# autonomousvision/ppo.cpp

Measured on AMD Instinct MI355X. Metric: env steps/sec (SPS), HalfCheetah-v5 num_envs=4096 at 1/2/4/8 MI355X, higher is better.
Workload: dtype f32

## Files before the change

### include/ppo_hip.h

```cpp
#ifndef PPO_HIP_H
#define PPO_HIP_H

#include <stddef.h>
#include <stdint.h>

#include "ppo_layout.h"

#ifdef __cplusplus
extern "C" {
#endif

typedef struct ppo_ctx ppo_t;

typedef struct ppo_hip_config {
  int net_kind;
  int obs_dim, act_dim;
  int hidden;
  int num_envs;
  int num_steps;
  int num_minibatches;
  int update_epochs;
  float gamma, gae_lambda;
  float clip_coef, ent_coef, vf_coef, max_grad_norm, adam_eps;
  int norm_adv, clip_vloss;
// ... 35 lines not shown
                             void* stream);
int ppo_get_value(ppo_t* ctx, int n, const float* x_dev, float* value_dev, void* stream);

int ppo_rollout_act(ppo_t* ctx, int step, int env_begin, int env_end, const float* next_obs_dev,
                    const float* next_done_dev, float* action_out_dev, void* stream);
int ppo_rollout_values(ppo_t* ctx, void* stream);
int ppo_rollout_reward(ppo_t* ctx, int step, int env_begin, int env_end, const float* reward_dev, void* stream);
int ppo_compute_gae(ppo_t* ctx, const float* next_obs_dev, const float* next_done_dev, int num_steps_collected,
                    void* stream);
int ppo_gae_from_values(ppo_t* ctx, const float* next_value_dev, const float* next_done_dev, int num_steps_collected,
                        void* stream);
int ppo_update(ppo_t* ctx, float lr, const int32_t* perms_dev, ppo_update_stats* stats);
int ppo_update_ex(ppo_t* ctx, float lr, int num_steps_collected, const int32_t* perms_dev, ppo_update_stats* stats);
int ppo_sync(ppo_t* ctx);
int ppo_debug_last_grad(ppo_t* ctx, float* host, long n);
int ppo_snapshot_state(ppo_t* ctx);
int ppo_read_snapshot(ppo_t* ctx, float* params_host, float* m_host, float* v_host, long n, long* step);
long ppo_iteration(const ppo_t* ctx);
int ppo_set_iteration(ppo_t* ctx, long iteration);
float* ppo_buffer(ppo_t* ctx, int which);

#define PPO_COMM_ID_BYTES 128
int ppo_comm_unique_id(char id_out[PPO_COMM_ID_BYTES]);
int ppo_comm_init(ppo_t* ctx, const char id[PPO_COMM_ID_BYTES], int rank, int world);
typedef int (*ppo_host_allreduce_fn)(float* host_buf, long n, int average, void* user);
int ppo_comm_init_host(ppo_t* ctx, int rank, int world, ppo_host_allreduce_fn fn, void* user);
int ppo_comm_destroy(ppo_t* ctx);
int ppo_comm_broadcast_params(ppo_t* ctx, int root);
int ppo_comm_allreduce(ppo_t* ctx, float* buf_dev, long n, int average);
enum { PPO_COMM_NONE = 0, PPO_COMM_RCCL = 1, PPO_COMM_HOST = 2 };
int ppo_comm_info(const ppo_t* ctx, int* kind, int* rank, int* world);
int ppo_get_device(const ppo_t* ctx, int* device, char* pci_bus_id, int len);
int ppo_kernel_info(const ppo_t* ctx, char* buf, int len);

int ppo_set_device(int device);
int ppo_device_count(int* n);
int ppo_dev_malloc(void** p, size_t bytes);
int ppo_dev_free(void* p);
int ppo_memcpy_h2d(void* dst_dev, const void* src_host, size_t bytes);
int ppo_memcpy_d2h(void* dst_host, const void* src_dev, size_t bytes);
int ppo_memset_dev(void* dst_dev, int value, size_t bytes);
int ppo_device_sync(void);

int ppo_profile_enable(ppo_t* ctx, int on);
int ppo_profile_read(ppo_t* ctx, double* ms, long* count, int cap);
const char* ppo_profile_name(int id);
int ppo_profile_reset(ppo_t* ctx);

#ifdef __cplusplus
}
#endif
#endif
```

### ppo.cpp_amd/csrc/ppo_capi.hip

```cpp
#include <hip/hip_runtime.h>
#include <rccl/rccl.h>

#include <dlfcn.h>
#include <link.h>
#include <unistd.h>

#include <algorithm>
#include <atomic>
#include <cmath>
#include <cstdio>
#include <cstdlib>
#include <cstring>
#include <mutex>
#include <string>
#include <vector>

#include "../../include/ppo_hip.h"
#include "../../include/ppo_synth_env.h"
#include "../../include/ppo_env_wrappers.h"
#include "ppo_kernels.hpp"

static thread_local std::string g_err;
static int fail(const std::string& msg, int code = -1) {
  g_err = msg;
// ... 112 lines not shown
  int upd32_mix = 0;
  bool use_upd2 = false;
  int rollout_kernel = 0;
  int upd2_split = 0;
  float* Z1 = nullptr;
  UpdGeoOut upd = {};
  int upd_nblk = 0;
  size_t lds_bytes = 0;
  int wlds_off = 0;
  float* dwslab[4] = {};
  int nchunks = 1, rows_per_chunk = 64, dw_slices = 1;
  float* normout = nullptr;
  float* gnpart = nullptr;
  float* cs_sq = nullptr;
  unsigned* cs_cnt = nullptr;
  int gn_fold = 0;
  float* mbstats = nullptr;
  float* snap = nullptr;
  hipEvent_t snap_ev = nullptr;
  hipStream_t snap_stream = nullptr;
  long snap_step = 0;
  long adam_step = 0;
  long iteration = 0;
  ncclComm_t comm = nullptr;
  ppo_host_allreduce_fn host_ar = nullptr;
  void* host_user = nullptr;
  std::vector<float> host_stage;
  int world = 1, rank = 0;
  int act_kernel = 0;
  int upd_trunk_mask = 3, upd_sched = 1;
  int dw_fused = 1;
  int dw_dma = 1;
  int dw_bx = 0;
  int rollout_mode = PPO_ROLLOUT_AUTO;
  int gradstep = 0;
  unsigned* gs_bar = nullptr;
  unsigned gs_count = 0;
  int update_graph = 0;
  bool update_graph_auto = false;
  hipGraphExec_t upd_exec = nullptr;
  const int32_t* upd_exec_perms = nullptr;
  long upd_calls = 0;
  float* sched = nullptr;
  float* sched_host[2] = {};
  hipEvent_t sched_ev[2] = {};
  int sched_flip = 0;
  float* beta_store = nullptr;
  unsigned prof_mask = 0;
  std::mutex prof_mu;
  std::vector<ProfEvent> pending;
  std::vector<hipEvent_t> free_events;
  double prof_ms[PK_COUNT] = {};
  long prof_cnt[PK_COUNT] = {};
};

static hipEvent_t prof_event(ppo_t* c) {
  if (!c->free_events.empty()) {
    hipEvent_t e = c->free_events.back();
    c->free_events.pop_back();
    return e;
  }
  hipEvent_t e;
  (void)hipEventCreate(&e);
  return e;
}
struct ProfScope {
// ... 28 lines not shown
    c->free_events.push_back(p.a);
    c->free_events.push_back(p.b);
  }
  c->pending.clear();
}

static hipStream_t S(ppo_t* c, void* s) { return s ? (hipStream_t)s : c->stream; }
static void comm_detach(ppo_t* c);

template <typename T>
static int dmalloc(T** p, size_t n) {
  if (n == 0) n = 1;
  hipError_t e = hipMalloc((void**)p, n * sizeof(T));
  if (e != hipSuccess) return fail(std::string("hipMalloc: ") + hipGetErrorString(e), -2);
  (void)hipMemset(*p, 0, n * sizeof(T));
  return 0;
}

struct CreateOptions {
  int upd_kernel = 0;
  int act_kernel = 0;
  int dw_fused = 1;
  int rollout = PPO_ROLLOUT_AUTO;
  int gradstep = 0;
  int gradnorm = -1;
  int dw_rows = 0;
  int dw_slices = 0;
  int dw_dma = 1;
  int dw_bx = -1;
  int gae_scan = -1;
  int values_mfma = -1;
  int upd_split = 0;
  int h1_handoff = -1;
  int update_graph = -1;
  int rollout_kernel = 0;
  int upd2_split = -1;
  int upd_mfma = 0;
};
static constexpr int kUpd2SplitAuto = 0;
static constexpr int kDwBxAuto = 6;
static constexpr int kUpdBxAuto = 1;
static constexpr int kUpd2BxAuto = 1;
static constexpr int kGaeScanMinT = 512;
static int kUpdSplitAuto(int M) { (void)M; return 1; }
static constexpr bool kH1RecomputeAuto = false;
static constexpr int kUpdGraphAutoRows = 4096;
static constexpr int kGradnormFoldAuto = 0;
static int parse_create_options(const char* opts, CreateOptions* o) {
  if (!opts) return 0;
  std::string s(opts);
  size_t pos = 0;
  while (pos < s.size()) {
    size_t end = s.find(',', pos);
    if (end == std::string::npos) end = s.size();
    const std::string kv = s.substr(pos, end - pos);
    pos = end + 1;
    if (kv.empty()) continue;
    const size_t eq = kv.find('=');
    if (eq == std::string::npos) return fail("ppo_create_ex: option without '=': " + kv);
    const std::string k = kv.substr(0, eq), v = kv.substr(eq + 1);
    if (k == "upd_kernel" && (v == "auto" || v == "fwdbwd")) o->upd_kernel = v == "fwdbwd";
    else if (k == "act_kernel" && (v == "auto" || v == "2" || v == "4")) o->act_kernel = v == "auto" ? 0 : v[0] - '0';
    else if (k == "dw_fused" && (v == "0" || v == "1")) o->dw_fused = v[0] - '0';
    else if (k == "rollout" && (v == "auto" || v == "per_step"))
      o->rollout = v == "auto" ? PPO_ROLLOUT_AUTO : PPO_ROLLOUT_PER_STEP;
    else if (k == "gradstep" && (v == "fused" || v == "split")) o->gradstep = v == "fused";
    else if (k == "gradnorm" && (v == "auto" || v == "slices" || v == "fold")) o->gradnorm = v == "auto" ? -1 : v == "fold";
    else if (k == "dw_rows" && !v.empty() && v.size() <= 5 && v.find_first_not_of("0123456789") == std::string::npos &&
             atoi(v.c_str()) % 16 == 0 && atoi(v.c_str()) >= 16 && atoi(v.c_str()) <= 65536)
      o->dw_rows = atoi(v.c_str());
    else if (k == "dw_slices" && (v == "1" || v == "2")) o->dw_slices = v[0] - '0';
    else if (k == "dw_dma" && (v == "0" || v == "1")) o->dw_dma = v[0] - '0';
    else if (k == "gae" && (v == "auto" || v == "serial" || v == "scan")) o->gae_scan = v == "auto" ? -1 : v == "scan";
    else if (k == "h1_handoff" && (v == "auto" || v == "store" || v == "recompute"))
      o->h1_handoff = v == "auto" ? -1 : v == "recompute";
    else if (k == "upd_split" && (v == "auto" || v == "1" || v == "2" || v == "4" || v == "8"))
      o->upd_split = v == "auto" ? 0 : v[0] - '0';
    else if (k == "values_mfma" && (v == "auto" || v == "f32" || v == "bx6"))
      o->values_mfma = v == "auto" ? -1 : v == "f32" ? 0 : 6;
    else if (k == "dw_mfma" && (v == "auto" || v == "f32" || v == "bf16x9" || v == "bf16x8" || v == "bf16x6"))
      o->dw_bx = v == "auto" ? -1 : v == "f32" ? 0 : v == "bf16x9" ? 9 : v == "bf16x8" ? 8 : 6;
    else if (k == "update_graph" && (v == "auto" || v == "0" || v == "1")) o->update_graph = v == "auto" ? -1 : v[0] - '0';
    else if (k == "rollout_kernel" && (v == "auto" || v == "mfma" || v == "valu"))
      o->rollout_kernel = v == "auto" ? 0 : v == "mfma" ? 1 : 2;
    else if (k == "upd2_split" && (v == "auto" || v == "0" || v == "2" || v == "3")) o->upd2_split = v == "auto" ? -1 : v[0] - '0';
    else if (k == "upd_mfma" && (v == "auto" || v == "16" || v == "32" || v == "mix" || v == "bx6"))
      o->upd_mfma = v == "auto" ? 0 : v == "mix" ? 1 : v == "bx6" ? 6 : atoi(v.c_str());
    else return fail("ppo_create_ex: unknown option or value: " + kv);
  }
  return 0;
}

extern "C" int ppo_create(const ppo_hip_config* cfg, int device, ppo_t** out) {
  return ppo_create_ex(cfg, device, nullptr, out);
}

extern "C" int ppo_create_ex(const ppo_hip_config* cfg, int device, const char* options, ppo_t** out) {
  if (!cfg || !out) return fail("ppo_create: null argument");
  CreateOptions opt;
  if (parse_create_options(options, &opt)) return -1;
  if (int rc = ppo_runtime_check()) return rc;
  ppo_layout L;
  if (ppo_layout_init(&L, cfg->net_kind, cfg->obs_dim, cfg->act_dim, cfg->hidden) != 0)
    return fail("ppo_create: bad net kind / dims");
  if (cfg->hidden != 64 && cfg->hidden != 256) return fail("ppo_create: hidden must be 64 or 256");
  if (cfg->act_dim > 20) return fail("ppo_create: act_dim > 20 not supported");
  if (cfg->num_envs <= 0 || cfg->num_steps <= 0 || cfg->num_minibatches <= 0 || cfg->update_epochs <= 0)
    return fail("ppo_create: sizes must be positive");
// ... 164 lines not shown
      if (opt.upd_split > 1) {
        ppo_destroy(c);
        return fail("ppo_create: upd_split > 1 needs the fused k_upd + k_dwf path (hidden 256, obs_dim <= 32)");
      }
      S = 1;
    }
    while (S > 1 && c->M < S * 32 * 64) S /= 2;
    c->msplit = S;
    c->Mq = S == 1 ? c->M : (((c->M + S - 1) / S + 31) & ~31);
    while (c->msplit > 1 && (long)(c->msplit - 1) * c->Mq >= c->M) --c->msplit;
  }
  for (int k = 0; k < 2; ++k)
    rc |= dmalloc(&c->slab[k], (size_t)c->msplit * std::max(c->nblk, c->upd_nblk) * c->sg[k].size);
  c->wlds_off = 4 * std::max(c->sg[0].size, c->sg[1].size);
  c->wlds_off = (c->wlds_off + 63) & ~63;
  c->lds_bytes = ((size_t)c->wlds_off + 2 * (size_t)H * 16) * sizeof(float);
  c->dw_slices = dw_slices(c->Mq, H, OP, true);
  if (opt.dw_slices && H == 256 && OP <= 32) c->dw_slices = opt.dw_slices;
  c->rows_per_chunk = std::max(64, (((c->Mq + 128 / c->dw_slices - 1) / (128 / c->dw_slices)) + 15) & ~15);
  if (c->use_upd2) c->rows_per_chunk = std::max(32, (((c->M + 255) / 256) + 31) & ~31);
  if (opt.dw_rows && (!c->use_upd2 || opt.dw_rows % 32 == 0)) c->rows_per_chunk = opt.dw_rows;
  c->nchunks = (c->Mq + c->rows_per_chunk - 1) / c->rows_per_chunk;
  {
    const bool rc_ok = c->use_upd && !c->use_upd2 && !c->use_upd32 && cfg->net_kind == PPO_NET_LN_BETA && H == 256 &&
                       OP <= 32 && c->dw_fused && c->dw_dma && c->dw_bx;
    if (opt.h1_handoff == 1 && !rc_ok) {
      ppo_destroy(c);
      return fail("ppo_create: h1_handoff=recompute needs the LayerNorm-Beta agent at hidden 256 (obs_dim <= 32) with "
                  "the fused split-bf16 dW (dw_mfma bf16x6/x8/x9)");
    }
    c->h1_recomp = rc_ok && (opt.h1_handoff == 1 || (opt.h1_handoff < 0 && kH1RecomputeAuto));
    if (c->h1_recomp)
      for (int k = 0; k < 2; ++k) rc |= dmalloc(&c->LNS[k], 2 * (size_t)c->M);
  }
  for (int k = 0; k < 2; ++k) rc |= dmalloc(&c->dwslab[k], (size_t)c->msplit * c->nchunks * (H * H + H * OP));
  if (c->upd2_split) rc |= dmalloc(&c->Z1, Mr * 128);
  rc |= dmalloc(&c->normout, 2 + PPO_LAYOUT_MAX_TENSORS + 2);
  rc |= dmalloc(&c->gnpart, (size_t)PPO_LAYOUT_MAX_TENSORS * PPO_GN_SPLIT);
  rc |= dmalloc(reinterpret_cast<float**>(&c->gs_bar), 1);
  rc |= dmalloc(&c->cs_sq, (size_t)c->K.size / 64 + 2 * PPO_MAX_SEGS + 64);
  rc |= dmalloc(reinterpret_cast<float**>(&c->cs_cnt), PPO_MAX_SEGS);
  rc |= dmalloc(&c->mbstats, (size_t)8 * EP * c->nmb);
  if (rc) {
    ppo_destroy(c);
    return -2;
  }
  if (fwdbwd_set_lds(c->K, c->lds_bytes) != 0) {
    ppo_destroy(c);
    return fail("ppo_create: cannot set LDS size for the fused update kernel");
  }
  HIP_TRY(hipDeviceSynchronize());
  *out = c;
  return 0;
}

extern "C" int ppo_destroy(ppo_t* c) {
  if (!c) return 0;
  (void)hipSetDevice(c->device);
  if (c->stream) (void)hipStreamSynchronize(c->stream);
  prof_drain(c);
  for (auto e : c->free_events) (void)hipEventDestroy(e);
  float* ptrs[] = {c->P, c->G, c->Am, c->Av, c->W2T[0], c->W2T[1], c->WSW[0], c->WSW[1], c->next_value, c->advstats, c->advsq, c->Xn, c->Z1,
                   c->normout, c->gnpart, c->mbstats, c->beta_store, reinterpret_cast<float*>(c->gs_bar), c->cs_sq,
                   reinterpret_cast<float*>(c->cs_cnt)};
  for (float* p : ptrs)
    if (p) (void)hipFree(p);
// ... 373 lines not shown
  u.Xn = c->Xn;
  u.Z1 = c->Z1;
  u.actn_off = c->upd.actn_off;
  u.acc_off = c->upd.acc_off;
  u.spar_off = c->upd.spar_off;
  u.hw_global = c->upd.hw_global;
  u.trunk_mask = c->upd_trunk_mask;
  u.sched = c->upd_sched;
  u.h1_skip = c->h1_recomp;
#ifdef PPO_DIAG
  {
    static const int hot = [] { const char* e = getenv("PPO_UPD2_HOT"); return e ? atoi(e) : 0; }();
    u.hot = hot;
  }
#endif
  const int nblk = c->use_upd ? c->upd_nblk : c->nblk;
  const int nsrow = c->msplit * nblk;
  for (int k = 0; k < 2; ++k) {
    u.H1[k] = c->H1[k];
    u.LNS[k] = c->LNS[k];
    u.DZ1[k] = c->DZ1[k];
    u.DZ2[k] = c->DZ2[k];
    u.slab[k] = c->slab[k];
  }
  DwArgs dw;
  memset(&dw, 0, sizeof(dw));
  dw.M = M;
  dw.rows_per_chunk = c->rows_per_chunk;
  dw.slices = c->dw_slices;
  dw.fused = c->dw_fused;
  dw.dma = c->dw_dma;
  dw.bx = c->dw_dma ? c->dw_bx : 0;
  dw.h1_recompute = c->h1_recomp;
  dw.kl1 = (c->K.O == 16 * (c->K.OP / 16 - 1) + 1) ? 1 : 4;
  dw.xn = c->Xn;
  dw.obs = c->buf[PPO_BUF_OBS];
  dw.O = c->K.O;
  dw.obs_n = B * c->K.O;
  dw.slab_stride = (long)H * H + (long)H * OP;
  for (int k = 0; k < 2; ++k) {
    dw.dz2[k] = c->DZ2[k];
    dw.h1[k] = c->H1[k];
    dw.lns[k] = c->LNS[k];
    dw.w1sw[k] = c->WSW[k];
    dw.b1[k] = c->P + c->K.tr[k].b1;
    dw.g1[k] = c->P + c->K.tr[k].g1;
    dw.be1[k] = c->P + c->K.tr[k].be1;
    dw.dz1[k] = c->DZ1[k];
    dw.slab[k] = c->dwslab[k];
  }
  ColsumArgs cs;
  memset(&cs, 0, sizeof(cs));
  int ns = 0;
  long maxlen = 0;
  auto seg = [&](const float* src, long stride, int count, int len, float* dst, float scale) {
    cs.seg[ns++] = ColsumSeg{src, dst, stride, count, len, scale};
    maxlen = std::max(maxlen, (long)len);
  };
  const bool ln = cfg.net_kind == PPO_NET_LN_BETA;
  for (int k = 0; k < 2; ++k) {
    const TrunkDev& T = c->K.tr[k];
    seg(c->dwslab[k], dw.slab_stride, c->msplit * c->nchunks, H * H, c->G + T.W2, 1.f);
    seg(c->dwslab[k] + (long)H * H, dw.slab_stride, c->msplit * c->nchunks, H * OP, c->G + T.W1, 1.f);
    const SmallGradLayout& g = c->sg[k];
    const float* sl = c->slab[k];
    seg(sl + g.b1, g.size, nsrow, H, c->G + T.b1, 1.f);
// ... 353 lines not shown
    *kind = PPO_COMM_RCCL;
    NCCL_TRY(ncclCommCount(c->comm, world));
    NCCL_TRY(ncclCommUserRank(c->comm, rank));
  } else if (c->host_ar) {
    *kind = PPO_COMM_HOST;
    *rank = c->rank;
    *world = c->world;
  } else {
    *kind = PPO_COMM_NONE;
    *rank = c->rank;
    *world = c->world;
  }
  return 0;
}

extern "C" int ppo_get_device(const ppo_t* c, int* device, char* pci_bus_id, int len) {
  if (!c || !device) return fail("ppo_get_device: null argument");
  *device = c->device;
  if (pci_bus_id && len > 0) HIP_TRY(hipDeviceGetPCIBusId(pci_bus_id, len, c->device));
  return 0;
}

extern "C" int ppo_kernel_info(const ppo_t* c, char* buf, int len) {
  if (!c || !buf || len <= 0) return fail("ppo_kernel_info: null argument");
  std::string upd = c->use_upd2    ? (c->upd2_split ? "k_l1g+k_upd2" : c->upd_bx ? "k_upd2/bx6" : "k_upd2/f32")
                    : c->use_upd32 ? (c->upd32_mix ? "k_upd32/mix" : "k_upd32")
                    : c->use_upd   ? (c->upd_bx ? "k_upd/bx6" : "k_upd/f32")
                                   : "k_fwdbwd";
  if (c->use_upd && !c->use_upd2 && c->upd.hw_global) upd += "/hwg";
  const int H = c->K.H, OP = c->K.OP;
  const bool fused = c->dw_fused && H == 256 && (OP == 16 || OP == 32);
  const std::string bxs = c->dw_bx ? "/bf16x" + std::to_string(c->dw_bx) : "/f32";
  std::string dw = c->use_upd2 ? (c->dw_dma && OP == 384 && c->K.O % 4 == 0 ? "k_dw2_dma" + bxs : "k_dw2")
                   : fused ? (!c->dw_dma ? "k_dwf" : c->dw_bx ? "k_dwf_bx/bf16x" + std::to_string(c->dw_bx) + (c->h1_recomp ? "/h1rc" : "")
                                                        : "k_dwf_dma/f32")
                   : (c->dw_dma && H == 256 && OP == 112) ? "k_dw_dma" + bxs
                                                          : "k_dw";
  const std::string vals = rollout_supported(c->K) != 0 ? "k_act" : c->values_bx ? "k_vbx/bx6"
                           : c->K.kind == PPO_NET_TANH_NORMAL ? "k_values4/f32" : "k_values/f32";
  const std::string s = "update=" + upd + " dw=" + dw + " values=" + vals +
                        (c->gn_fold && !c->gradstep ? " norm=k_colsum" : c->gradstep ? " norm=k_gradstep" : " norm=k_gradnorm");
  snprintf(buf, (size_t)len, "%s", s.c_str());
  return 0;
}

extern "C" int ppo_set_device(int d) {
  if (int rc = ppo_runtime_check()) return rc;
  int ndev = 0;
  HIP_TRY(hipGetDeviceCount(&ndev));
  if (d < 0 || d >= ndev)
    return fail("ppo_set_device: device " + std::to_string(d) + " requested but " + std::to_string(ndev) +
                " HIP device(s) are visible");
  HIP_TRY(hipSetDevice(d));
  return 0;
}
extern "C" int ppo_device_count(int* n) { HIP_TRY(hipGetDeviceCount(n)); return 0; }
extern "C" int ppo_dev_malloc(void** p, size_t bytes) {
  if (int rc = ppo_runtime_check()) return rc;
  HIP_TRY(hipMalloc(p, bytes ? bytes : 1));
  HIP_TRY(hipMemset(*p, 0, bytes ? bytes : 1));
  HIP_TRY(hipDeviceSynchronize());
  return 0;
}
extern "C" int ppo_dev_free(void* p) {
  HIP_TRY(hipDeviceSynchronize());
  HIP_TRY(hipFree(p));
  return 0;
}
extern "C" int ppo_memcpy_h2d(void* d, const void* h, size_t n) {
  HIP_TRY(hipDeviceSynchronize());
  HIP_TRY(hipMemcpy(d, h, n, hipMemcpyHostToDevice));
  HIP_TRY(hipDeviceSynchronize());
  return 0;
}
extern "C" int ppo_memcpy_d2h(void* h, const void* d, size_t n) {
  HIP_TRY(hipDeviceSynchronize());
// ... 315 lines not shown
```

### ppo.cpp_amd/csrc/ppo_kernels.hip

```cpp
#include "ppo_agent.hpp"
#include "ppo_kernels.hpp"
#include "ppo_wrap.hpp"

#include <algorithm>
#include <cstdlib>
#include <type_traits>
#ifndef PPO_DWD_AUX
#define PPO_DWD_AUX 0
#endif

template <int H, int KIND, int NTO>
__global__ __launch_bounds__(64) void k_act(ActArgs a) {
  constexpr int NT = H / 16;
  const int lane = threadIdx.x, j = lane & 15, g = lane >> 4;
  const int trunk = blockIdx.y;
  const int row = blockIdx.x * 16 + j;
  const bool valid = row < a.n;
  const PackedLayout& K = a.K;
  const float* __restrict__ P = a.P;
  const float* xrow = valid ? a.x + (size_t)row * a.ldx : nullptr;
  const long env = a.env_base + row;
  const long srow = (long)a.store_step * a.E + env;

  f4 xin[NTO];
// ... 1324 lines not shown
#pragma unroll
        for (int e = 0; e < 8; ++e) x[e] = sb[oDZ1 + e * LDH + w1row + l32];
        a1s = split3(x);
        const float* xb = lds + (sI % NBUF) * STG + oXN + (8 * hs) * LDX;
#pragma unroll
        for (int e = 0; e < 8; ++e) x[e] = l32 < OP ? xb[e * LDX + l32] : 0.0f;
        b1s = split3(x);
      }
    }
#pragma unroll
    for (int v = 0; v < TIW; ++v) {
      float x[8];
#pragma unroll
      for (int e = 0; e < 8; ++e) x[e] = hb[e * LDH + (wi * TIW + v) * 32 + l32];
      const Split3 bs = split3(x);
#pragma unroll
      for (int u = 0; u < TOW; ++u) acc[u][v] = mfma_split<NP>(as[u], bs, acc[u][v]);
    }
    if (w1_wave) acc1 = mfma_split<NP>(a1s, b1s, acc1);
  }
  float* out = a.slab[trunk] + (size_t)blockIdx.x * a.slab_stride;
#pragma unroll
  for (int r = 0; r < 16; ++r) {
    const int orow = (r & 3) + 8 * (r >> 2) + 4 * hs;
#pragma unroll
    for (int u = 0; u < TOW; ++u)
#pragma unroll
      for (int v = 0; v < TIW; ++v)
        dw_st(out + (size_t)(obase + (wo * TOW + u) * 32 + orow) * H + (wi * TIW + v) * 32 + l32, acc[u][v][r]);
    if (w1_wave && l32 < OP) dw_st(out + (size_t)H * H + (size_t)(w1row + orow) * OP + l32, acc1[r]);
  }
}

typedef __attribute__((address_space(1))) float gfl;
typedef __attribute__((address_space(1))) unsigned gu32;
PPO_DEV void colsum_fold(const ColsumArgs& a, int sgi, int b, float ss) {
  const int lane = threadIdx.x & 63;
#pragma unroll
  for (int m = 8; m >= 1; m >>= 1) ss += __shfl_xor(ss, m, 64);
  unsigned ticket = 0;
  if (lane == 0) {
    __hip_atomic_store((gfl*)(a.sq + b), ss, __ATOMIC_RELAXED, __HIP_MEMORY_SCOPE_AGENT);
    asm volatile("s_waitcnt vmcnt(0)" ::: "memory");
    ticket = __hip_atomic_fetch_add((gu32*)(a.cnt + sgi), 1u, __ATOMIC_RELAXED, __HIP_MEMORY_SCOPE_AGENT);
  }
  ticket = __shfl(ticket, 0, 64);
  const int t0 = a.tile0[sgi], n = a.tile0[sgi + 1] - t0;
  if ((int)ticket != n - 1) return;
  __builtin_amdgcn_fence(__ATOMIC_ACQUIRE, "wavefront");
  float acc = 0.f;
  for (int k0 = 0; k0 < n; k0 += 1024) {
    float v[16];
#pragma unroll
    for (int j = 0; j < 16; ++j) {
      const int k = k0 + lane + 64 * j;
      v[j] = __hip_atomic_load((gfl*)(a.sq + t0 + min(k, n - 1)), __ATOMIC_RELAXED, __HIP_MEMORY_SCOPE_AGENT);
    }
#pragma unroll
    for (int j = 0; j < 16; ++j) acc += (k0 + lane + 64 * j < n) ? v[j] : 0.f;
  }
#pragma unroll
  for (int m = 32; m >= 1; m >>= 1) acc += __shfl_xor(acc, m, 64);
  if (lane < PPO_GN_SPLIT) a.part[a.seg_t[sgi] * PPO_GN_SPLIT + lane] = lane == 0 ? acc : 0.f;
  if (lane == 0) __hip_atomic_store((gu32*)(a.cnt + sgi), 0u, __ATOMIC_RELAXED, __HIP_MEMORY_SCOPE_AGENT);
}

// ... 679 lines not shown
    return hipFuncSetAttribute(
               (const void*)k_fwdbwd<decltype(H_)::value, decltype(KIND_)::value, decltype(NTO_)::value>,
               hipFuncAttributeMaxDynamicSharedMemorySize, (int)lds_bytes) == hipSuccess
               ? 0
               : -2;
  });
}

template <int H, int OP>
static int launch_dw_t(const DwArgs& a, int nchunks, size_t lds, hipStream_t s) {
  auto k = k_dw<H, OP>;
  static bool attr = false;
  if (!attr) {
    if (hipFuncSetAttribute((const void*)k, hipFuncAttributeMaxDynamicSharedMemorySize, (int)lds) != hipSuccess) return -2;
    attr = true;
  }
  hipLaunchKernelGGL(k, dim3(nchunks, 2), dim3(512), lds, s, a);
  return 0;
}

size_t dw_lds_bytes(int H, int OP) {
  const int KS = 16;
  const int m = std::max(H, OP) + 4;
  return (size_t)2 * (KS * (H + 4) + KS * m) * sizeof(float);
}

template <int H, int OP, int NSL>
static int launch_dwf_t(const DwArgs& a0, int nchunks, hipStream_t s) {
  DwArgs a = a0;
#ifdef PPO_DIAG
  static const int hot = [] { const char* e = getenv("PPO_DW_HOT"); return e ? atoi(e) : 0; }();
  a.hot = hot;
#endif
  if (a.bx && (long)a.M * H < (1L << 29)) {
    const bool rc = a.h1_recompute != 0;
    auto k = rc ? (a.bx == 9 ? k_dwf_bx<H, OP, NSL, 9, true> : a.bx == 8 ? k_dwf_bx<H, OP, NSL, 8, true>
                                                              : k_dwf_bx<H, OP, NSL, 6, true>)
                : (a.bx == 9 ? k_dwf_bx<H, OP, NSL, 9> : a.bx == 8 ? k_dwf_bx<H, OP, NSL, 8> : k_dwf_bx<H, OP, NSL, 6>);
    const size_t lds = (size_t)(rc ? DwbxGeo<H, OP, true>::total : DwbxGeo<H, OP, false>::total) * sizeof(float);
    static_assert(DwbxGeo<H, OP, true>::total * sizeof(float) <= 160 * 1024, "k_dwf_bx (H1 recompute) LDS");
    static bool attr[6] = {false, false, false, false, false, false};
    const int ai = (a.bx == 9 ? 2 : a.bx == 8 ? 1 : 0) + (rc ? 3 : 0);
    if (!attr[ai]) {
      if (hipFuncSetAttribute((const void*)k, hipFuncAttributeMaxDynamicSharedMemorySize, (int)lds) != hipSuccess) return -2;
      attr[ai] = true;
    }
    hipLaunchKernelGGL(k, dim3(nchunks, 2, NSL), dim3(512), lds, s, a);
    return 0;
  }
  if (a.dma && (long)a.M * H < (1L << 29)) {
    auto k = k_dwf_dma<H, OP, NSL>;
    constexpr size_t lds = (size_t)3 * (3 * 16 * H + 16 * OP) * sizeof(float);
    static bool attr = false;
    if (!attr) {
      if (hipFuncSetAttribute((const void*)k, hipFuncAttributeMaxDynamicSharedMemorySize, (int)lds) != hipSuccess) return -2;
      attr = true;
    }
    hipLaunchKernelGGL(k, dim3(nchunks, 2, NSL), dim3(512), lds, s, a);
    return 0;
  }
  auto k = k_dwf<H, OP, NSL>;
  constexpr size_t lds = (size_t)2 * (3 * 16 * (H + 4) + 16 * (OP + 4)) * sizeof(float);
  static bool attr = false;
  if (!attr) {
    if (hipFuncSetAttribute((const void*)k, hipFuncAttributeMaxDynamicSharedMemorySize, (int)lds) != hipSuccess) return -2;
    attr = true;
// ... 111 lines not shown
```

### ppo.cpp_amd/csrc/ppo_kernels.hpp

```cpp
#pragma once

#include <hip/hip_runtime.h>
#include <stdint.h>

#include <string>

#include "ppo_device.hpp"
#include "ppo_packed.hpp"

#include "../../include/ppo_hip.h"

struct ActArgs {
  const float* P;
  PackedLayout K;
  int n;
  const float* x;
  int ldx;
  int mode;
  int need_actor;
  const float* action_in;
  uint64_t seed;
  int rank;
  long env_base;
  long step_id;
  float* action_out;
  float* logprob_out;
  float* entropy_out;
  float* value_out;
  int store_step;
  int E;
  const float* next_done;
  float *s_obs, *s_actions, *s_logp, *s_dones, *s_values;
  int kernel;
  const float* WSW[2];
  int skip_critic;
};

PPO_DEV_HOST inline long sw_index(int r, int c, int ncols) {
  return ((long)((r >> 4) * (ncols >> 4) + (c >> 4)) * 64 + ((c & 15) >> 2) * 16 + (r & 15)) * 4 + (c & 3);
}
PPO_DEV_HOST inline long sw_size(int H, int OP) { return (long)H * OP + 2L * H * H; }

PPO_DEV_HOST inline void split3_bits(float x, uint16_t (&pc)[3]) {
  const uint32_t u = __builtin_bit_cast(uint32_t, x);
  const float r = x - __builtin_bit_cast(float, u & 0xffff0000u);
  const uint32_t v = __builtin_bit_cast(uint32_t, r);
  const float l = r - __builtin_bit_cast(float, v & 0xffff0000u);
  pc[0] = (uint16_t)(u >> 16);
  pc[1] = (uint16_t)(v >> 16);
  pc[2] = (uint16_t)(__builtin_bit_cast(uint32_t, l) >> 16);
}
PPO_DEV_HOST inline long bx_index(int r, int c, int ncols, int p) {
  const int lane = (r & 15) + 16 * ((c & 15) >> 2), e = 4 * ((c >> 4) & 1) + (c & 3);
  return ((((long)(r >> 4) * (ncols >> 5) + (c >> 5)) * 3 + p) * 64 + lane) * 8 + e;
}
PPO_DEV_HOST inline long bx_size(int H) { return 3L * H * H; }
PPO_DEV_HOST inline long bx_w1_size(int H, int OP) { return 3L * H * OP / 2; }
PPO_DEV_HOST inline long bx_region(int H, int OP) { return H == 256 ? bx_size(H) : H == 64 ? bx_w1_size(H, OP) : 0; }

struct UpdArgs {
  const float* P;
  const float* W2T[2];
  const float* WSW[2];
  PackedLayout K;
  SmallGradLayout sg[2];
  int M;
  int tiles_per_block;
  int wlds_off;
  const int32_t* perm;
  const float *obs, *actions, *logp, *adv, *ret, *val;
  long rows_n, obs_n;
  const float* adv_stats;
  float clip_coef, ent_coef, vf_coef, inv_m;
  int clip_vloss, norm_adv;
  float* Xn;
  float* H1[2];
  float* DZ1[2];
  float* DZ2[2];
  float* slab[2];
  int actn_off, acc_off, spar_off;
  int hw_global;
  float* Z1;
  int trunk_mask;
  int sched;
  int hot;
  int bx;
  int h1_skip;
  float* LNS[2];
};

#define PPO_UPD_MAXA 24
struct UpdGeoOut {
  size_t lds_bytes;
  int actn_off, acc_off, spar_off, rows;
  int hw_global;
};

struct DwArgs {
  const float* dz2[2];
  const float* h1[2];
  const float* dz1[2];
  const float* xn;
  const int32_t* perm;
  const float* obs;
  long obs_n;
  int O;
  float* slab[2];
  long slab_stride;
  int M;
  int rows_per_chunk;
  int fused;
  int slices;
  int dma;
  int bx;
  int hot;
  int h1_recompute, kl1;
  const float* lns[2];
  const float* w1sw[2];
  const float *b1[2], *g1[2], *be1[2];
};
inline int dw_slices(int M, int H, int OP, bool fused) { return (fused && H == 256 && OP <= 32 && M <= 32768) ? 2 : 1; }

struct ColsumSeg {
  const float* src;
  float* dst;
  long stride;
  int count;
  int len;
  float scale;
};
#define PPO_MAX_SEGS 40
struct ColsumArgs {
  ColsumSeg seg[PPO_MAX_SEGS];
  int tile0[PPO_MAX_SEGS + 1];
  int nseg;
  int fold;
  int seg_t[PPO_MAX_SEGS];
  float* sq;
  unsigned* cnt;
  float* part;
};

struct NormArgs {
  const float* grad;
  int nt;
  int off[PPO_LAYOUT_MAX_TENSORS];
  int len[PPO_LAYOUT_MAX_TENSORS];
// ... 149 lines not shown
```

### ppo.cpp_amd/ppo_amd/__init__.py

```python
from __future__ import annotations

import ctypes as C
import os
import subprocess
from dataclasses import dataclass, field

import numpy as np

try:
    import torch
except ImportError:
    torch = None

HERE = os.path.dirname(os.path.abspath(__file__))
PKG_ROOT = os.path.dirname(HERE)
LIB_PATH = os.environ.get("PPO_HIP_LIB") or os.path.join(PKG_ROOT, "lib", "libppo_hip.so")

PPO_NET_TANH_NORMAL = 0
PPO_NET_LN_BETA = 1
PPO_SAMPLE, PPO_MEAN, PPO_GIVEN = 0, 1, 2
(BUF_OBS, BUF_ACTIONS, BUF_LOGPROBS, BUF_REWARDS, BUF_DONES, BUF_VALUES, BUF_ADVANTAGES,
 BUF_RETURNS) = range(8)
MAX_T = 32

# ... 110 lines not shown
    ("ppo_create_ex", _I, [C.POINTER(HipConfig), _I, C.c_char_p, C.POINTER(_VP)]),
    ("ppo_destroy", _I, [_VP]),
    ("ppo_get_layout", _I, [_VP, C.POINTER(Layout)]),
    ("ppo_stream", _VP, [_VP]),
    ("ppo_load_params", _I, [_VP, _FP, _L]),
    ("ppo_save_params", _I, [_VP, _FP, _L]),
    ("ppo_save_adam", _I, [_VP, _FP, _FP, _L, C.POINTER(_L)]),
    ("ppo_load_adam", _I, [_VP, _FP, _FP, _L, _L]),
    ("ppo_get_action_and_value", _I, [_VP, _I, _FP, _I, _FP, _L, _L, _FP, _FP, _FP, _FP, _VP]),
    ("ppo_get_value", _I, [_VP, _I, _FP, _FP, _VP]),
    ("ppo_rollout_act", _I, [_VP, _I, _I, _I, _FP, _FP, _FP, _VP]),
    ("ppo_rollout_values", _I, [_VP, _VP]),
    ("ppo_rollout_reward", _I, [_VP, _I, _I, _I, _FP, _VP]),
    ("ppo_compute_gae", _I, [_VP, _FP, _FP, _I, _VP]),
    ("ppo_gae_from_values", _I, [_VP, _FP, _FP, _I, _VP]),
    ("ppo_update", _I, [_VP, _F, _VP, C.POINTER(UpdateStats)]),
    ("ppo_update_ex", _I, [_VP, _F, _I, _VP, C.POINTER(UpdateStats)]),
    ("ppo_sync", _I, [_VP]),
    ("ppo_debug_last_grad", _I, [_VP, _FP, _L]),
    ("ppo_snapshot_state", _I, [_VP]),
    ("ppo_read_snapshot", _I, [_VP, _FP, _FP, _FP, _L, C.POINTER(_L)]),
    ("ppo_iteration", _L, [_VP]),
    ("ppo_set_iteration", _I, [_VP, _L]),
    ("ppo_buffer", _VP, [_VP, _I]),
    ("ppo_comm_unique_id", _I, [C.c_char_p]),
    ("ppo_comm_init", _I, [_VP, C.c_char_p, _I, _I]),
    ("ppo_comm_init_host", _I, [_VP, _I, _I, C.c_void_p, _VP]),
    ("ppo_comm_destroy", _I, [_VP]),
    ("ppo_comm_broadcast_params", _I, [_VP, _I]),
    ("ppo_comm_allreduce", _I, [_VP, _FP, _L, _I]),
    ("ppo_comm_info", _I, [_VP, C.POINTER(_I), C.POINTER(_I), C.POINTER(_I)]),
    ("ppo_get_device", _I, [_VP, C.POINTER(_I), C.c_char_p, _I]),
    ("ppo_kernel_info", _I, [_VP, C.c_char_p, _I]),
    ("ppo_set_device", _I, [_I]),
    ("ppo_device_count", _I, [C.POINTER(_I)]),
    ("ppo_dev_malloc", _I, [C.POINTER(_VP), _SZ]),
    ("ppo_dev_free", _I, [_VP]),
    ("ppo_memcpy_h2d", _I, [_VP, _VP, _SZ]),
    ("ppo_memcpy_d2h", _I, [_VP, _VP, _SZ]),
    ("ppo_memset_dev", _I, [_VP, _I, _SZ]),
    ("ppo_device_sync", _I, []),
    ("ppo_profile_enable", _I, [_VP, _I]),
    ("ppo_profile_read", _I, [_VP, C.POINTER(C.c_double), C.POINTER(_L), _I]),
    ("ppo_profile_name", C.c_char_p, [_I]),
    ("ppo_profile_reset", _I, [_VP]),
    ("psyn_create", _I, [_I, _I, _I, C.POINTER(_VP)]),
    ("psyn_destroy", _I, [_VP]),
    ("psyn_reset", _I, [_VP, _I, _FP, _FP, _VP]),
    ("psyn_step", _I, [_VP, _I, _I, _FP, _F, _F, _FP, _FP, _FP, _VP]),
    ("psyn_episode_stats", _I, [_VP, C.POINTER(_F), C.POINTER(_F), C.POINTER(_F)]),
    ("psyn_episode_stats_begin", _I, [_VP, _VP]),
    ("psyn_episode_stats_end", _I, [_VP, C.POINTER(_F), C.POINTER(_F), C.POINTER(_F)]),
    ("ppo_rollout_synth", _I, [_VP, _VP, _FP, _FP, _FP, _FP]),
    ("psyn_set_action_space", _I, [_VP, _F, _F]),
    ("ppo_set_rollout_mode", _I, [_VP, _I]),
    ("psyn_action_space", _I, [_VP, C.POINTER(_F), C.POINTER(_F)]),
    ("psyn_attach_wrappers", _I, [_VP, _VP]),
    ("pwrap_create", _I, [_I, _I, _F, C.POINTER(_VP)]),
    ("pwrap_destroy", _I, [_VP]),
    ("pwrap_reset", _I, [_VP, _I, _I, _FP, _VP]),
    ("pwrap_step", _I, [_VP, _I, _I, _FP, _FP, _FP, _FP, _VP]),
    ("pwrap_read_state", _I, [_VP, _FP, _L]),
    ("ppo_carla_create", _I, [C.POINTER(CarlaConfig), _I, C.POINTER(_VP)]),
    ("ppo_carla_create_ex", _I, [C.POINTER(CarlaConfig), _I, C.c_char_p, C.POINTER(_VP)]),
    ("ppo_carla_destroy", _I, [_VP]),
    ("ppo_carla_get_layout", _I, [_VP, C.POINTER(CarlaLayout)]),
# ... 733 lines not shown
```

Baseline: 34.53 million.

## Add split-once staged dW kernel storing bf16x3 pieces in swizzled LDS

Adds a new fused weight-gradient kernel, enabled by default when the fused split-bf16 dW path applies. Each source value is split into hi/mid/lo bf16 pieces once when staged into a double-buffered, bank-swizzled LDS image. MFMA operands are then read back with transposing LDS loads, so the kernel no longer re-splits operands for each use. The loop also interleaves global prefetch with the MMA work via sched_group_barrier. The cost is much larger LDS use per block, which can lower occupancy, plus new swizzle-indexing code that needs to be correct.

Result: faster. 35.17 million (median of 6 runs) (+1.8%).

```diff
diff --git a/include/ppo_hip.h b/include/ppo_hip.h
--- a/include/ppo_hip.h
+++ b/include/ppo_hip.h
@@ -91,6 +91,7 @@
 int ppo_comm_info(const ppo_t* ctx, int* kind, int* rank, int* world);
 int ppo_get_device(const ppo_t* ctx, int* device, char* pci_bus_id, int len);
 int ppo_kernel_info(const ppo_t* ctx, char* buf, int len);
+int ppo_dw_image_offset(int row, int col);
 
 int ppo_set_device(int device);
 int ppo_device_count(int* n);
diff --git a/ppo.cpp_amd/csrc/ppo_capi.hip b/ppo.cpp_amd/csrc/ppo_capi.hip
--- a/ppo.cpp_amd/csrc/ppo_capi.hip
+++ b/ppo.cpp_amd/csrc/ppo_capi.hip
@@ -168,6 +168,7 @@
   int dw_fused = 1;
   int dw_dma = 1;
   int dw_bx = 0;
+  int dw_so = 0;
   int rollout_mode = PPO_ROLLOUT_AUTO;
   int gradstep = 0;
   unsigned* gs_bar = nullptr;
@@ -262,6 +263,7 @@
   int values_mfma = -1;
   int upd_split = 0;
   int h1_handoff = -1;
+  int dw_stage = -1;
   int update_graph = -1;
   int rollout_kernel = 0;
   int upd2_split = -1;
@@ -274,6 +276,7 @@
 static constexpr int kGaeScanMinT = 512;
 static int kUpdSplitAuto(int M) { (void)M; return 1; }
 static constexpr bool kH1RecomputeAuto = false;
+static constexpr bool kDwSplitOnceAuto = true;
 static constexpr int kUpdGraphAutoRows = 4096;
 static constexpr int kGradnormFoldAuto = 0;
 static int parse_create_options(const char* opts, CreateOptions* o) {
@@ -304,6 +307,8 @@
     else if (k == "gae" && (v == "auto" || v == "serial" || v == "scan")) o->gae_scan = v == "auto" ? -1 : v == "scan";
     else if (k == "h1_handoff" && (v == "auto" || v == "store" || v == "recompute"))
       o->h1_handoff = v == "auto" ? -1 : v == "recompute";
+    else if (k == "dw_stage" && (v == "auto" || v == "dma" || v == "split_once"))
+      o->dw_stage = v == "auto" ? -1 : v == "split_once";
     else if (k == "upd_split" && (v == "auto" || v == "1" || v == "2" || v == "4" || v == "8"))
       o->upd_split = v == "auto" ? 0 : v[0] - '0';
     else if (k == "values_mfma" && (v == "auto" || v == "f32" || v == "bx6"))
@@ -534,6 +539,14 @@
     c->h1_recomp = rc_ok && (opt.h1_handoff == 1 || (opt.h1_handoff < 0 && kH1RecomputeAuto));
     if (c->h1_recomp)
       for (int k = 0; k < 2; ++k) rc |= dmalloc(&c->LNS[k], 2 * (size_t)c->M);
+    const bool so_ok = !c->use_upd2 && H == 256 && (OP == 16 || OP == 32) && c->dw_fused && c->dw_dma && c->dw_bx &&
+                       !c->h1_recomp;
+    if (opt.dw_stage == 1 && !so_ok) {
+      ppo_destroy(c);
+      return fail("ppo_create: dw_stage=split_once needs the fused split-bf16 dW (hidden 256, obs_dim <= 32, dw_mfma "
+                  "bf16x6/x8/x9) with h1_handoff=store");
+    }
+    c->dw_so = so_ok && (opt.dw_stage == 1 || (opt.dw_stage < 0 && kDwSplitOnceAuto));
   }
   for (int k = 0; k < 2; ++k) rc |= dmalloc(&c->dwslab[k], (size_t)c->msplit * c->nchunks * (H * H + H * OP));
   if (c->upd2_split) rc |= dmalloc(&c->Z1, Mr * 128);
@@ -973,6 +986,7 @@
   dw.dma = c->dw_dma;
   dw.bx = c->dw_dma ? c->dw_bx : 0;
   dw.h1_recompute = c->h1_recomp;
+  dw.split_once = c->dw_so;
   dw.kl1 = (c->K.O == 16 * (c->K.OP / 16 - 1) + 1) ? 1 : 4;
   dw.xn = c->Xn;
   dw.obs = c->buf[PPO_BUF_OBS];
@@ -1392,7 +1406,7 @@
   const bool fused = c->dw_fused && H == 256 && (OP == 16 || OP == 32);
   const std::string bxs = c->dw_bx ? "/bf16x" + std::to_string(c->dw_bx) : "/f32";
   std::string dw = c->use_upd2 ? (c->dw_dma && OP == 384 && c->K.O % 4 == 0 ? "k_dw2_dma" + bxs : "k_dw2")
-                   : fused ? (!c->dw_dma ? "k_dwf" : c->dw_bx ? "k_dwf_bx/bf16x" + std::to_string(c->dw_bx) + (c->h1_recomp ? "/h1rc" : "")
+                   : fused ? (!c->dw_dma ? "k_dwf" : c->dw_bx ? "k_dwf_bx/bf16x" + std::to_string(c->dw_bx) + (c->h1_recomp ? "/h1rc" : c->dw_so ? "/split_once" : "")
                                                         : "k_dwf_dma/f32")
                    : (c->dw_dma && H == 256 && OP == 112) ? "k_dw_dma" + bxs
                                                           : "k_dw";
@@ -1402,6 +1416,10 @@
                         (c->gn_fold && !c->gradstep ? " norm=k_colsum" : c->gradstep ? " norm=k_gradstep" : " norm=k_gradnorm");
   snprintf(buf, (size_t)len, "%s", s.c_str());
   return 0;
+}
+
+extern "C" int ppo_dw_image_offset(int row, int col) {
+  return row < 0 || row >= 16 || col < 0 || col >= 256 || (col & 3) ? -1 : dwso_off(row, col);
 }
 
 extern "C" int ppo_set_device(int d) {
diff --git a/ppo.cpp_amd/csrc/ppo_kernels.hip b/ppo.cpp_amd/csrc/ppo_kernels.hip
--- a/ppo.cpp_amd/csrc/ppo_kernels.hip
+++ b/ppo.cpp_amd/csrc/ppo_kernels.hip
@@ -1380,6 +1380,200 @@
   }
 }
 
+template <int OP>
+struct DwsoGeo {
+  static constexpr int PIECE = 16 * 256 * 2;
+  static constexpr int SRC = 3 * PIECE;
+  static constexpr int oXN = 3 * SRC;
+  static constexpr int XPIECE = 16 * 32 * 2;
+  static constexpr int IMG = oXN + 3 * XPIECE;
+  static constexpr int total = 2 * IMG;
+  static constexpr int SPILL = 2 * XPIECE + 64 * 8;
+  static constexpr int lds = total + SPILL;
+};
+#ifndef PPO_DWSO_SGB
+#define PPO_DWSO_SGB 1
+#endif
+#ifndef PPO_DWSO_PRIO
+#define PPO_DWSO_PRIO 0
+#endif
+#ifndef PPO_DWSO_RELOAD
+#define PPO_DWSO_RELOAD 0
+#endif
+typedef short dwso_v4s __attribute__((ext_vector_type(4)));
+typedef unsigned u32x2 __attribute__((ext_vector_type(2)));
+PPO_DEV u32x2 lds_read_tr16(const unsigned char* p) {
+  return __builtin_bit_cast(u32x2, __builtin_amdgcn_ds_read_tr16_b64_v4i16((__attribute__((address_space(3))) dwso_v4s*)p));
+}
+template <int STRIDE>
+PPO_DEV Split3 dwso_operand(const unsigned char* p0, const unsigned char* p1) {
+  Split3 s;
+  const u32x2 h0 = lds_read_tr16(p0), h1 = lds_read_tr16(p1);
+  const u32x2 m0 = lds_read_tr16(p0 + STRIDE), m1 = lds_read_tr16(p1 + STRIDE);
+  const u32x2 l0 = lds_read_tr16(p0 + 2 * STRIDE), l1 = lds_read_tr16(p1 + 2 * STRIDE);
+  s.hi = u32x4{h0[0], h0[1], h1[0], h1[1]};
+  s.mid = u32x4{m0[0], m0[1], m1[0], m1[1]};
+  s.lo = u32x4{l0[0], l0[1], l1[0], l1[1]};
+  return s;
+}
+template <int STRIDE>
+PPO_DEV void dwso_split_store(unsigned char* p, f4 x) {
+  unsigned h0, m0, l0, h1, m1, l1;
+  split3_pair(x[0], x[1], h0, m0, l0);
+  split3_pair(x[2], x[3], h1, m1, l1);
+  *reinterpret_cast<u32x2*>(p) = u32x2{h0, h1};
+  *reinterpret_cast<u32x2*>(p + STRIDE) = u32x2{m0, m1};
+  *reinterpret_cast<u32x2*>(p + 2 * STRIDE) = u32x2{l0, l1};
+}
+template <int H, int OP, int NSL, int NP>
+__global__ __launch_bounds__(512) void k_dwf_so(DwArgs a) {
+  extern __shared__ __attribute__((aligned(16))) unsigned char ldsb[];
+  using GE = DwsoGeo<OP>;
+  constexpr int KS = 16;
+  static_assert(H == 256 && (OP == 16 || OP == 32), "k_dwf_so geometry");
+  constexpr int NXI = KS * OP / 256;
+  constexpr int TOW = 2 / NSL, TIW = 4;
+  static_assert(NSL == 1 || NSL == 2, "k_dwf slices");
+  static_assert(NP == 6 || NP == 8 || NP == 9, "k_dwf_so passes");
+  static_assert(GE::lds <= 160 * 1024, "k_dwf_so LDS");
+  const int tid = threadIdx.x, lane = tid & 63, wave = __builtin_amdgcn_readfirstlane(tid >> 6), l32 = lane & 31,
+            hs = lane >> 5;
+  const int wo = wave & 3, wi = wave >> 2;
+  const int trunk = blockIdx.y, slice = NSL > 1 ? (int)blockIdx.z : 0;
+  const int obase = slice * (H / NSL);
+  const bool w1_wave = NSL == 1 || wave < 8 / NSL;
+  const int w1row = obase + wave * 32;
+  const long m0 = (long)blockIdx.x * a.rows_per_chunk;
+  const long m1 = min((long)a.M, m0 + a.rows_per_chunk);
+  if (m0 >= m1) return;
+  const uint32_t rows_bytes = (uint32_t)((long)a.M * H * 4), xn_bytes = (uint32_t)((long)a.M * OP * 4);
+  const PBuf bdz2 = make_pbuf(a.dz2[trunk], (int)(rows_bytes / 4)), bh1 = make_pbuf(a.h1[trunk], (int)(rows_bytes / 4));
+  const PBuf bdz1 = make_pbuf(a.dz1[trunk], (int)(rows_bytes / 4));
+  const PBuf bxn = make_pbuf(a.xn, (int)(xn_bytes / 4));
+  const int srow = 2 * wave + ((lane >> 3) & 1), scol = 32 * (lane >> 4) + 4 * (lane & 7);
+  const int xe = wave * 256 + lane * 4, xrow = xe / OP, xcol = xe - xrow * OP;
+  const bool xw = wave < NXI;
+  const int wofs = dwso_off(srow, scol);
+  const int xwofs = GE::oXN + 64 * xrow + 2 * xcol;
+  f4 pv[6], px = {0.f, 0.f, 0.f, 0.f};
+  auto load_src = [&](long mb, int s3) {
+    if (s3 < 3) {
+      const long row = mb + srow;
+#pragma unroll
+      for (int i = 0; i < 2; ++i) {
+        const uint32_t voff = row < m1 ? (uint32_t)((row * H + scol + 128 * i) * 4) : 0xFFFFFFF0u;
+        pv[2 * s3 + i] = __builtin_bit_cast(
+            f4, __builtin_amdgcn_raw_buffer_load_b128((s3 == 0 ? bdz2 : s3 == 1 ? bh1 : bdz1).r, voff, 0, PPO_DW_AUX));
+      }
+    } else {
+      const long xr = mb + xrow;
+      const uint32_t voff = xw && xr < m1 ? (uint32_t)((xr * OP + xcol) * 4) : 0xFFFFFFF0u;
+      px = __builtin_bit_cast(f4, __builtin_amdgcn_raw_buffer_load_b128(bxn.r, voff, 0, PPO_DW_AUX));
+    }
+  };
+  auto load = [&](long mb) {
+#pragma unroll
+    for (int s3 = 0; s3 < 4; ++s3) load_src(mb, s3);
+  };
+  auto put = [&](unsigned char* img, int s3) {
+    if (s3 < 3) {
+      dwso_split_store<GE::PIECE>(img + s3 * GE::SRC + wofs, pv[2 * s3]);
+      dwso_split_store<GE::PIECE>(img + s3 * GE::SRC + wofs + 4096, pv[2 * s3 + 1]);
+    } else {
+      dwso_split_store<GE::XPIECE>(xw ? img + xwofs : ldsb + GE::total + 8 * lane, px);
+    }
+  };
+  const int rq = (lane >> 2) & 3, rc = 16 * ((lane >> 4) & 1) + 4 * (lane & 3);
+  const int rofs0 = dwso_off(8 * hs + rq, rc), rofs1 = dwso_off(8 * hs + 4 + rq, rc);
+  const int xrofs = GE::oXN + 64 * (8 * hs + rq) + 2 * rc;
+  f16v acc[TOW][TIW], acc1;
+#pragma unroll
+  for (int r = 0; r < 16; ++r) {
+    acc1[r] = 0.0f;
+#pragma unroll
+    for (int u = 0; u < TOW; ++u)
+#pragma unroll
+      for (int v = 0; v < TIW; ++v) acc[u][v][r] = 0.0f;
+  }
+  if constexpr (OP < 32) {
+    constexpr int NZ = 3 * GE::XPIECE / 4;
+    for (int i = tid; i < 2 * NZ; i += 512)
+      *reinterpret_cast<unsigned*>(ldsb + (i >= NZ ? GE::IMG : 0) + GE::oXN + 4 * (i >= NZ ? i - NZ : i)) = 0u;
+    lds_barrier();
+  }
+  const int nst = (int)((m1 - m0 + KS - 1) / KS);
+#if PPO_DWSO_PRIO
+  if (wave >= 4) __builtin_amdgcn_s_setprio(1);
+#endif
+  load(m0);
+#pragma unroll
+  for (int s3 = 0; s3 < 4; ++s3) put(ldsb, s3);
+  load(m0 + KS);
+  lds_barrier();
+  for (int sI = 0; sI < nst; ++sI) {
+    const unsigned char* ib = ldsb + (sI & 1) * GE::IMG;
+    unsigned char* ob = ldsb + ((sI + 1) & 1) * GE::IMG;
+    if (w1_wave) {
+      const Split3 a1s = dwso_operand<GE::PIECE>(ib + 2 * GE::SRC + dwso_off(0, w1row) + rofs0,
+                                                 ib + 2 * GE::SRC + dwso_off(0, w1row) + rofs1);
+      const Split3 b1s = dwso_operand<GE::XPIECE>(ib + xrofs, ib + xrofs + 256);
+      acc1 = mfma_split<NP>(a1s, b1s, acc1);
+    }
+    Split3 as[TOW];
+#pragma unroll
+    for (int u = 0; u < TOW; ++u) {
+      const int c = dwso_off(0, obase + (wo * TOW + u) * 32);
+      as[u] = dwso_operand<GE::PIECE>(ib + c + rofs0, ib + c + rofs1);
+    }
+    const int cb = GE::SRC + dwso_off(0, wi * TIW * 32);
+    const long mb2 = m0 + (long)(sI + 2) * KS;
+#if PPO_DWSO_SGB
+    Split3 bs = dwso_operand<GE::PIECE>(ib + cb + rofs0, ib + cb + rofs1);
+#pragma unroll
+    for (int v = 0; v < TIW; ++v) {
+      __builtin_amdgcn_sched_barrier(0);
+      Split3 bn = bs;
+      if (v + 1 < TIW) bn = dwso_operand<GE::PIECE>(ib + cb + 512 * (v + 1) + rofs0, ib + cb + 512 * (v + 1) + rofs1);
+#pragma unroll
+      for (int u = 0; u < TOW; ++u) acc[u][v] = mfma_split<NP>(as[u], bs, acc[u][v]);
+      put(ob, v);
+      bs = bn;
+      constexpr int NM = TOW * NP;
+#pragma unroll
+      for (int g = 0; g < NM; ++g) {
+        __builtin_amdgcn_sched_group_barrier(0x008, 1, 0);
+        __builtin_amdgcn_sched_group_barrier(0x002, (52 + NM - 1) / NM, 0);
+        __builtin_amdgcn_sched_group_barrier(0x080, (12 + NM - 1) / NM, 0);
+      }
+      __builtin_amdgcn_sched_barrier(0);
+      if (PPO_DWSO_RELOAD) load_src(mb2, v);
+    }
+#else
+#pragma unroll
+    for (int v = 0; v < TIW; ++v) {
+      const Split3 bs = dwso_operand<GE::PIECE>(ib + cb + 512 * v + rofs0, ib + cb + 512 * v + rofs1);
+#pragma unroll
+      for (int u = 0; u < TOW; ++u) acc[u][v] = mfma_split<NP>(as[u], bs, acc[u][v]);
+      put(ob, v);
+      if (PPO_DWSO_RELOAD) load_src(mb2, v);
+    }
+#endif
+    if (!PPO_DWSO_RELOAD) load(mb2);
+    lds_barrier();
+  }
+  float* out = a.slab[trunk] + (size_t)blockIdx.x * a.slab_stride;
+#pragma unroll
+  for (int r = 0; r < 16; ++r) {
+    const int orow = (r & 3) + 8 * (r >> 2) + 4 * hs;
+#pragma unroll
+    for (int u = 0; u < TOW; ++u)
+#pragma unroll
+      for (int v = 0; v < TIW; ++v)
+        dw_st(out + (size_t)(obase + (wo * TOW + u) * 32 + orow) * H + (wi * TIW + v) * 32 + l32, acc[u][v][r]);
+    if (w1_wave && l32 < OP) dw_st(out + (size_t)H * H + (size_t)(w1row + orow) * OP + l32, acc1[r]);
+  }
+}
+
 typedef __attribute__((address_space(1))) float gfl;
 typedef __attribute__((address_space(1))) unsigned gu32;
 PPO_DEV void colsum_fold(const ColsumArgs& a, int sgi, int b, float ss) {
@@ -2125,6 +2319,18 @@
   static const int hot = [] { const char* e = getenv("PPO_DW_HOT"); return e ? atoi(e) : 0; }();
   a.hot = hot;
 #endif
+  if (a.bx && a.split_once && !a.h1_recompute && (long)a.M * H < (1L << 29)) {
+    auto k = a.bx == 9 ? k_dwf_so<H, OP, NSL, 9> : a.bx == 8 ? k_dwf_so<H, OP, NSL, 8> : k_dwf_so<H, OP, NSL, 6>;
+    constexpr size_t lds = DwsoGeo<OP>::lds;
+    static bool attr[3] = {false, false, false};
+    const int ai = a.bx == 9 ? 2 : a.bx == 8 ? 1 : 0;
+    if (!attr[ai]) {
+      if (hipFuncSetAttribute((const void*)k, hipFuncAttributeMaxDynamicSharedMemorySize, (int)lds) != hipSuccess) return -2;
+      attr[ai] = true;
+    }
+    hipLaunchKernelGGL(k, dim3(nchunks, 2, NSL), dim3(512), lds, s, a);
+    return 0;
+  }
   if (a.bx && (long)a.M * H < (1L << 29)) {
     const bool rc = a.h1_recompute != 0;
     auto k = rc ? (a.bx == 9 ? k_dwf_bx<H, OP, NSL, 9, true> : a.bx == 8 ? k_dwf_bx<H, OP, NSL, 8, true>
diff --git a/ppo.cpp_amd/csrc/ppo_kernels.hpp b/ppo.cpp_amd/csrc/ppo_kernels.hpp
--- a/ppo.cpp_amd/csrc/ppo_kernels.hpp
+++ b/ppo.cpp_amd/csrc/ppo_kernels.hpp
@@ -55,6 +55,10 @@
   return ((((long)(r >> 4) * (ncols >> 5) + (c >> 5)) * 3 + p) * 64 + lane) * 8 + e;
 }
 PPO_DEV_HOST inline long bx_size(int H) { return 3L * H * H; }
+PPO_DEV_HOST inline constexpr int dwso_off(int row, int col) {
+  return 4096 * (col >> 7) + 2048 * (row >> 3) + 512 * ((col >> 5) & 3) + 64 * (row & 7) +
+         16 * (((col >> 3) & 3) ^ ((row >> 2) & 3)) + 8 * ((col >> 2) & 1);
+}
 PPO_DEV_HOST inline long bx_w1_size(int H, int OP) { return 3L * H * OP / 2; }
 PPO_DEV_HOST inline long bx_region(int H, int OP) { return H == 256 ? bx_size(H) : H == 64 ? bx_w1_size(H, OP) : 0; }
 
@@ -113,6 +117,7 @@
   int slices;
   int dma;
   int bx;
+  int split_once;
   int hot;
   int h1_recompute, kl1;
   const float* lns[2];
diff --git a/ppo.cpp_amd/ppo_amd/__init__.py b/ppo.cpp_amd/ppo_amd/__init__.py
--- a/ppo.cpp_amd/ppo_amd/__init__.py
+++ b/ppo.cpp_amd/ppo_amd/__init__.py
@@ -166,6 +166,7 @@
     ("ppo_comm_info", _I, [_VP, C.POINTER(_I), C.POINTER(_I), C.POINTER(_I)]),
     ("ppo_get_device", _I, [_VP, C.POINTER(_I), C.c_char_p, _I]),
     ("ppo_kernel_info", _I, [_VP, C.c_char_p, _I]),
+    ("ppo_dw_image_offset", _I, [_I, _I]),
     ("ppo_set_device", _I, [_I]),
     ("ppo_device_count", _I, [C.POINTER(_I)]),
     ("ppo_dev_malloc", _I, [C.POINTER(_VP), _SZ]),
```
